# starlingonearth/MASt3R-SLAM-Quality-dualTSDF

Hardware: AMD Instinct MI355X
Metric: SLAM frames/sec (infer+match+TSDF+GN) @512x384 (higher is better)
Workload: dtype bf16

## Files before the change

mast3r-slam-quality-dualtsdf_amd/csrc/gn.hip:

```cpp
#include "common.h"
#include "sim3.h"

namespace mslam {

constexpr int kAcc = 35;
constexpr int kEdgeConst = 16;
constexpr int kPlanes = 8;
constexpr int kTile = 64;

struct GnState {
  int done;
  int iters;
  int chol_fail;
  float last_norm;
};

__device__ __forceinline__ int64_t ij_val(const int64_t* ii, const int64_t* jj, int E, int k) {
  return k < E ? ii[k] : jj[k - E];
}

__global__ __launch_bounds__(256) void gn_first_kernel(const int64_t* __restrict__ ii,
                                                       const int64_t* __restrict__ jj, int E,
                                                       int* __restrict__ first) {
  const int k = blockIdx.x * 256 + threadIdx.x;
  if (k >= 2 * E) return;
  const int64_t v = ij_val(ii, jj, E, k);
  int f = 1;
  for (int m = 0; m < k; m++)
    if (ij_val(ii, jj, E, m) == v) { f = 0; break; }
  first[k] = f;
}

__global__ __launch_bounds__(256) void gn_rank_kernel(const int64_t* __restrict__ ii,
                                                      const int64_t* __restrict__ jj, int E, int num_fix,
                                                      const int* __restrict__ first,
                                                      int* __restrict__ ii_edge, int* __restrict__ jj_edge,
                                                      int* __restrict__ ii_opt, int* __restrict__ jj_opt) {
  const int k = blockIdx.x * 256 + threadIdx.x;
  if (k >= 2 * E) return;
  const int64_t v = ij_val(ii, jj, E, k);
  int rank = 0;
  for (int m = 0; m < 2 * E; m++) rank += (first[m] && ij_val(ii, jj, E, m) < v) ? 1 : 0;
  if (k < E) { ii_edge[k] = rank; ii_opt[k] = rank - num_fix; }
  else { jj_edge[k - E] = rank; jj_opt[k - E] = rank - num_fix; }
}

__global__ void gn_edge_setup_kernel(const GnState* __restrict__ st, const float* __restrict__ Twc,
                                     const int* __restrict__ ii_edge, const int* __restrict__ jj_edge,
                                     int E, float* __restrict__ econst) {
  if (st->done) return;
  const int e = blockIdx.x * blockDim.x + threadIdx.x;
  if (e >= E) return;
  const Sim3f Ti = sim3_load(Twc + 8 * ii_edge[e]);
  const Sim3f Tj = sim3_load(Twc + 8 * jj_edge[e]);
  const Sim3f Tij = sim3_rel(Ti, Tj);
  float R[9];
  quat_to_mat(Tij.q, R);
  float* c = econst + (size_t)e * kEdgeConst;
#pragma unroll
  for (int k = 0; k < 9; k++) c[k] = Tij.s * R[k];
  c[9] = Tij.t[0]; c[10] = Tij.t[1]; c[11] = Tij.t[2];
  c[12] = c[13] = c[14] = c[15] = 0.0f;
}

__global__ __launch_bounds__(256) void gn_compact_kernel(
    const float* __restrict__ Xs, const float* __restrict__ Cs, const int* __restrict__ ii_edge,
    const int* __restrict__ jj_edge, const int64_t* __restrict__ idx_ii2jj,
    const uint8_t* __restrict__ valid_match, const float* __restrict__ Q, int num_points, int chunk_len,
    float C_thresh, float Q_thresh, float* __restrict__ stream, int* __restrict__ counts, int S, int slot_begin) {
  const int e = blockIdx.x / S, chunk = blockIdx.x - e * S;
  const int ix = ii_edge[e], jx = jj_edge[e];
  const float* __restrict__ Xi_base = Xs + (size_t)ix * num_points * 3;
  const float* __restrict__ Xj_base = Xs + (size_t)jx * num_points * 3;
  const float* __restrict__ Ci_base = Cs + (size_t)ix * num_points;
  const float* __restrict__ Cj_base = Cs + (size_t)jx * num_points;
  const int64_t* __restrict__ idx_e = idx_ii2jj + (size_t)e * num_points;
  const uint8_t* __restrict__ vm_e = valid_match + (size_t)e * num_points;
  const float* __restrict__ Q_e = Q + (size_t)e * num_points;
  float* __restrict__ slot = stream + ((size_t)(slot_begin + e) * S + chunk) * (size_t)chunk_len * kPlanes;
  __shared__ int wave_cnt[4];
  const int lane = threadIdx.x & 63, wid = threadIdx.x >> 6;
  const int k_begin = chunk * chunk_len;
  const int k_end = min(k_begin + chunk_len, num_points);
  int base = 0;
  for (int k0 = k_begin; k0 < k_end; k0 += 256) {
    const int k = k0 + (int)threadIdx.x;
    bool valid = false;
    long long ind = 0;
    float q = 0.0f;
    if (k < k_end) {
      const bool vm = vm_e[k] != 0;
      ind = vm ? idx_e[k] : 0;
      q = Q_e[k];
      const float ci = Ci_base[ind], cj = Cj_base[k];
      valid = vm & (q > Q_thresh) & (ci > C_thresh) & (cj > C_thresh);
    }
    const unsigned long long m = __ballot(valid);
    if (lane == 0) wave_cnt[wid] = __popcll(m);
    __syncthreads();
    int off = base;
    for (int w = 0; w < wid; w++) off += wave_cnt[w];
    const int total = wave_cnt[0] + wave_cnt[1] + wave_cnt[2] + wave_cnt[3];
    if (valid) {
      const int pos = off + __popcll(m & ((1ull << lane) - 1ull));
      slot[0 * (size_t)chunk_len + pos] = Xi_base[ind * 3 + 0];
      slot[1 * (size_t)chunk_len + pos] = Xi_base[ind * 3 + 1];
      slot[2 * (size_t)chunk_len + pos] = Xi_base[ind * 3 + 2];
      slot[3 * (size_t)chunk_len + pos] = Xj_base[(size_t)k * 3 + 0];
      slot[4 * (size_t)chunk_len + pos] = Xj_base[(size_t)k * 3 + 1];
      slot[5 * (size_t)chunk_len + pos] = Xj_base[(size_t)k * 3 + 2];
      slot[6 * (size_t)chunk_len + pos] = sqrtf(q);
      slot[7 * (size_t)chunk_len + pos] = __int_as_float((int)ind);
    }
    base += total;
    __syncthreads();
  }
  if (threadIdx.x == 0) counts[(slot_begin + e) * S + chunk] = base;
}

__device__ __forceinline__ float fast_rcp(float x) { return __builtin_amdgcn_rcpf(x); }
__device__ __forceinline__ float fast_rsq(float x) { return __builtin_amdgcn_rsqf(x); }

__device__ __forceinline__ float huber_w(float r) {
  return fminf(1.0f, 1.345f * fast_rcp(fabsf(r)));
}

template <unsigned NZ>
__device__ __forceinline__ void accum_row(float (&acc)[kAcc], const float (&x)[7], float w, float err) {
  const float we = w * err;
  int l = 0;
#pragma unroll
  for (int n = 0; n < 7; n++) {
    const float wx = w * x[n];
#pragma unroll
    for (int m = 0; m <= n; m++) {
      if (((NZ >> n) & 1u) && ((NZ >> m) & 1u)) acc[l] = fmaf(wx, x[m], acc[l]);
      l++;
    }
    if ((NZ >> n) & 1u) acc[28 + n] = fmaf(we, x[n], acc[28 + n]);
  }
}

struct GnParams {
  float sa_inv, sb_inv;
  float C_thresh, Q_thresh;
  int height, width;
  float border_lo, border_hi_u, border_hi_v;
  float z_eps;
  const float* K;
};

struct EdgeConst {
// ... 143 lines not shown
  }
  __syncthreads();
  if (threadIdx.x < kAcc) {
    const float s = (red[0][threadIdx.x] + red[1][threadIdx.x]) + (red[2][threadIdx.x] + red[3][threadIdx.x]);
    partial[((size_t)e * S + chunk) * kAcc + threadIdx.x] = s;
  }
}

__global__ __launch_bounds__(64) void gn_reduce_kernel(const GnState* __restrict__ st,
                                                       const float* __restrict__ partial, int S,
                                                       const float* __restrict__ Twc,
                                                       const int* __restrict__ ii_edge, int e0, int E,
                                                       float* __restrict__ Hs, float* __restrict__ gs) {
  if (st->done) return;
  const int e = blockIdx.x;
  __shared__ double B[7][7];
  __shared__ double u[7];
  __shared__ double M[7][7];
  __shared__ double MB[7][7];
  const int t = threadIdx.x;
  if (t < kAcc) {
    double s = 0.0;
    for (int c = 0; c < S; c++) s += (double)partial[((size_t)e * S + c) * kAcc + t];
    if (t < 28) {
      int n = 0, rem = t;
      while (rem > n) { rem -= n + 1; n++; }
      B[n][rem] = s;
      B[rem][n] = s;
    } else {
      u[t - 28] = s;
    }
  }
  if (t == 63) {
    const float* p = Twc + 8 * ii_edge[e];
    const double tx = p[0], ty = p[1], tz = p[2], x = p[3], y = p[4], z = p[5], w = p[6];
    const double sinv = 1.0 / (double)p[7];
    const double R[3][3] = {{1 - 2 * (y * y + z * z), 2 * (x * y - z * w), 2 * (x * z + y * w)},
                            {2 * (x * y + z * w), 1 - 2 * (x * x + z * z), 2 * (y * z - x * w)},
                            {2 * (x * z - y * w), 2 * (y * z + x * w), 1 - 2 * (x * x + y * y)}};
    for (int a = 0; a < 7; a++)
      for (int b = 0; b < 7; b++) M[a][b] = 0.0;
    for (int a = 0; a < 3; a++)
      for (int b = 0; b < 3; b++) {
        M[a][b] = sinv * R[a][b];
        M[3 + a][3 + b] = R[a][b];
      }
    for (int b = 0; b < 3; b++) {
      M[3][b] = sinv * (ty * R[2][b] - tz * R[1][b]);
      M[4][b] = sinv * (tz * R[0][b] - tx * R[2][b]);
      M[5][b] = sinv * (tx * R[1][b] - ty * R[0][b]);
      M[6][b] = sinv * (tx * R[0][b] + ty * R[1][b] + tz * R[2][b]);
    }
    M[6][6] = 1.0;
  }
  __syncthreads();
  if (t < 49) {
    const int a = t / 7, b = t % 7;
    double s = 0.0;
    for (int k = 0; k < 7; k++) s += M[a][k] * B[k][b];
    MB[a][b] = s;
  }
  __syncthreads();
  if (t < 49) {
    const int a = t / 7, b = t % 7;
    double s = 0.0;
    for (int k = 0; k < 7; k++) s += MB[a][k] * M[b][k];
    const float A = (float)s;
    const size_t o = (size_t)(e0 + e) * 49 + t;
    const size_t blk = (size_t)E * 49;
    Hs[o] = A;
    Hs[blk + o] = -A;
    Hs[2 * blk + o] = -A;
    Hs[3 * blk + o] = A;
  } else if (t < 56) {
    const int a = t - 49;
    double s = 0.0;
    for (int k = 0; k < 7; k++) s += M[a][k] * u[k];
    gs[(size_t)(e0 + e) * 7 + a] = -(float)s;
    gs[(size_t)E * 7 + (size_t)(e0 + e) * 7 + a] = (float)s;
  }
}

constexpr int kTab = 32;

__global__ __launch_bounds__(64) void gn_assemble_kernel(const GnState* __restrict__ st,
                                                         const float* __restrict__ Hs,
                                                         const float* __restrict__ gs,
                                                         const int* __restrict__ ii_opt,
                                                         const int* __restrict__ jj_opt, int E, int N,
                                                         int np, int ld, double* __restrict__ Haug,
                                                         int* __restrict__ tmin32) {
  if (st->done) return;
  const int br = blockIdx.x;
  const int lane = threadIdx.x;
  const int n = N * 7;
  if (br == N) {
    for (int r = n + lane; r < np; r += 64) {
      Haug[(size_t)r * ld + r] = 1.0;
      atomicMin(&tmin32[r >> 5], r);
    }
    if (lane == 0) tmin32[np >> 5] = 0;
    return;
  }
  int cmin = br;
  __shared__ double tab[kTab][49];
  __shared__ int tabcol[kTab];
  int ntab = 0;
  double bacc = 0.0;
  const int k7 = lane / 7, l7 = lane % 7;
  for (int blk = 0; blk < 4; blk++) {
    const int* rix = (blk < 2) ? ii_opt : jj_opt;
    const int* cix = (blk & 1) ? jj_opt : ii_opt;
    for (int e0 = 0; e0 < E; e0 += 64) {
      const int e = e0 + lane;
      const bool row_match = e < E && rix[e] == br;
      const int cj_l = row_match ? cix[e] : -1;
      unsigned long long m = __ballot(row_match);
      while (m) {
        const int b = __ffsll((long long)m) - 1;
        m &= m - 1;
        const int ee = e0 + b;
        if ((blk == 0 || blk == 2) && lane < 7)
          bacc += (double)gs[((size_t)(blk >> 1) * E + ee) * 7 + lane];
        const int cj = __shfl(cj_l, b, 64);
        if (cj < 0) continue;
        cmin = min(cmin, cj);
        const double v = lane < 49 ? (double)Hs[((size_t)blk * E + ee) * 49 + lane] : 0.0;
        const unsigned long long hit = __ballot(lane < ntab && tabcol[lane] == cj);
        int slot = hit ? __ffsll((long long)hit) - 1 : -1;
        if (slot < 0 && ntab < kTab) {
          slot = ntab++;
          if (lane == 0) tabcol[slot] = cj;
          if (lane < 49) tab[slot][lane] = 0.0;
          __builtin_amdgcn_wave_barrier();
        }
        if (lane < 49) {
          if (slot >= 0) tab[slot][lane] += v;
          else Haug[(size_t)(7 * br + k7) * ld + 7 * cj + l7] += v;
        }
      }
    }
  }
  __syncthreads();
  for (int s = 0; s < ntab; s++) {
    const int cj = tabcol[s];
    if (lane < 49) Haug[(size_t)(7 * br + k7) * ld + 7 * cj + l7] += tab[s][lane];
  }
  if (lane < 7) Haug[(size_t)np * ld + 7 * br + lane] = bacc;
  if (lane < 7) atomicMin(&tmin32[(7 * br + lane) >> 5], 7 * cmin);
}

using f64x4 = __attribute__((ext_vector_type(4))) double;

template <int NB>
__global__ __launch_bounds__(256) void chol_step_kernel(GnState* __restrict__ st, double* __restrict__ A,
                                                        double* __restrict__ Ldiag, int np, int ld, int j0,
                                                        const int* __restrict__ tmin32, int update, int clim) {
  if (st->done) return;
  constexpr int LS = NB + 2;
  constexpr int TS = kTile + 1;
  constexpr int DS = NB + 1;
  const int tj = blockIdx.x, ti = blockIdx.y;
  if (tj > ti) return;
  const int j1 = j0 + NB;
  const int r0 = j1 + ti * kTile, c0 = j1 + tj * kTile;
  if (r0 > np || c0 >= np || c0 >= clim) return;
  const bool has_update = update != 0;
  {
    const int last = np >> 5;
    const int fr = min(tmin32[min(r0 >> 5, last)], tmin32[min((r0 >> 5) + 1, last)]);
    const int fc = min(tmin32[min(c0 >> 5, last)], tmin32[min((c0 >> 5) + 1, last)]);
    if (tj != 0 && (fr >= j1 || fc >= j1)) return;
    if (tj == 0 && fr >= j1 + NB) return;
  }
  extern __shared__ double sh[];
  double* Li = sh;
  double* Lj = sh + kTile * LS;
  double* T = sh;
  double* D = sh + 2 * kTile * LS;
  double* dsave = D + NB * DS;
  double* rdiag = dsave + NB;
  __shared__ int fail;
  const int t = threadIdx.x;
  const int lane = t & 63, wid = t >> 6;
  const int wr = wid >> 1, wc = wid & 1;
  const int fcol = lane & 15, frow = lane >> 4;

  f64x4 acc[2][2];
#pragma unroll
  for (int m = 0; m < 2; m++)
#pragma unroll
    for (int n = 0; n < 2; n++)
#pragma unroll
      for (int g = 0; g < 4; g++) {
        const int r = r0 + 32 * wr + 16 * m + frow + 4 * g;
        const int c = c0 + 32 * wc + 16 * n + fcol;
        const bool in = r <= np && c < np && c <= r && c < clim;
        const double v = A[in ? (size_t)r * ld + c : (size_t)0];
        acc[m][n][g] = in ? v : 0.0;
      }
  if (has_update) {
    for (int k = t; k < kTile * NB; k += 256) {
      const int r = k / NB, q = k % NB;
      const double vi = A[(size_t)min(r0 + r, np) * ld + j0 + q];
      const double vj = A[(size_t)min(c0 + r, np) * ld + j0 + q];
      Li[r * LS + q] = (r0 + r <= np) ? vi : 0.0;
      Lj[r * LS + q] = (c0 + r < np) ? vj : 0.0;
    }
  }
  if (tj == 0) {
    for (int k = t; k < NB * NB; k += 256) {
      const int a = k / NB, b = k % NB;
      D[a * DS + b] = A[(size_t)(j1 + a) * ld + j1 + b];
    }
    if (t == 0) fail = 0;
  }
  __syncthreads();

  if (has_update) {
    if (tj == 0) {
      for (int k = t; k < NB * NB; k += 256) {
        const int a = k / NB, b = k % NB;
        if (b <= a) {
          double s = 0.0;
#pragma unroll 8
          for (int q = 0; q < NB; q++) s = fma(Lj[a * LS + q], Lj[b * LS + q], s);
          D[a * DS + b] -= s;
        }
      }
    }
    const int fi = lane & 15, fk = lane >> 4;
#pragma unroll 4
    for (int k4 = 0; k4 < NB; k4 += 4) {
      double a[2], b[2];
#pragma unroll
      for (int m = 0; m < 2; m++) {
        a[m] = -Li[(32 * wr + 16 * m + fi) * LS + k4 + fk];
        b[m] = Lj[(32 * wc + 16 * m + fi) * LS + k4 + fk];
      }
#pragma unroll
      for (int m = 0; m < 2; m++)
#pragma unroll
        for (int n = 0; n < 2; n++)
          acc[m][n] = __builtin_amdgcn_mfma_f64_16x16x4f64(a[m], b[n], acc[m][n], 0, 0, 0);
    }
  }

  if (tj != 0) {
    if (has_update) {
#pragma unroll
      for (int m = 0; m < 2; m++)
#pragma unroll
        for (int n = 0; n < 2; n++)
#pragma unroll
          for (int g = 0; g < 4; g++) {
            const int r = r0 + 32 * wr + 16 * m + frow + 4 * g;
            const int c = c0 + 32 * wc + 16 * n + fcol;
            if (r <= np && c < np && c <= r && c < clim) A[(size_t)r * ld + c] = acc[m][n][g];
          }
    }
    return;
  }

  __syncthreads();
#pragma unroll
  for (int m = 0; m < 2; m++)
#pragma unroll
    for (int n = 0; n < 2; n++)
#pragma unroll
      for (int g = 0; g < 4; g++) {
        const int rr = 32 * wr + 16 * m + frow + 4 * g;
        const int cc = 32 * wc + 16 * n + fcol;
        const int r = r0 + rr, c = c0 + cc;
        if (cc < NB) T[rr * TS + cc] = acc[m][n][g];
        else if (has_update && r <= np && c < np && c <= r && c < clim) A[(size_t)r * ld + c] = acc[m][n][g];
      }

  __syncthreads();
  for (int j = 0; j < NB; j++) {
    const double djj = D[j * DS + j];
    const bool ok = djj > 0.0;
    double d, rinv;
    if (djj > 1e-30 && djj < 1e30) {
      double r = (double)__builtin_amdgcn_rsqf((float)djj);
      const double h = 0.5 * djj;
      r = r * (1.5 - h * r * r);
      r = r * (1.5 - h * r * r);
      r = r * (1.5 - h * r * r);
      rinv = r;
      d = djj * r;
    } else {
      d = ok ? sqrt(djj) : 1.0;
      rinv = 1.0 / d;
    }
    if (t > j && t < NB) D[t * DS + j] *= rinv;
    if (t == j) {
      dsave[j] = d;
      rdiag[j] = rinv;
      if (!ok) fail = 1;
    }
    __syncthreads();
#pragma unroll
    for (int i = 0; i < NB * NB / 256; i++) {
      const int k = t + 256 * i;
      const int r = k / NB, c = k % NB;
      if (c > j && c <= r) D[r * DS + c] -= D[r * DS + j] * D[c * DS + j];
    }
    __syncthreads();
  }
  if (ti == 0) {
    if (fail && t == 0) st->chol_fail = 1;
    double* Ld = Ldiag + (size_t)(j1 / NB) * NB * NB;
    for (int k = t; k < NB * NB; k += 256) {
      const int a = k / NB, b = k % NB;
      Ld[k] = (b < a) ? D[a * DS + b] : (b == a ? dsave[a] : 0.0);
    }
  }

  if (t < kTile) {
    const int r = r0 + t;
    const bool in_diag = (ti == 0) && (t < NB);
    if (r <= np && !in_diag) {
      double x[NB];
#pragma unroll
      for (int c = 0; c < NB; c++) x[c] = T[t * TS + c];
#pragma unroll
      for (int c = 0; c < NB; c++) {
        double s = x[c];
#pragma unroll
        for (int k = 0; k < c; k++) s -= x[k] * D[c * DS + k];
        x[c] = s * rdiag[c];
      }
#pragma unroll
      for (int c = 0; c < NB; c++) T[t * TS + c] = x[c];
    }
  }
  __syncthreads();
  for (int k = t; k < kTile * NB; k += 256) {
    const int rr = k / NB, c = k % NB;
    const int r = r0 + rr;
    const bool in_diag = (ti == 0) && (rr < NB);
    if (r <= np && !in_diag) A[(size_t)r * ld + j1 + c] = T[rr * TS + c];
  }
}

__global__ __launch_bounds__(256) void chol_outer_kernel(const GnState* __restrict__ st, double* __restrict__ A, int np,
                                                         int ld, int J0, int W, const int* __restrict__ tmin32) {
  if (st->done) return;
  constexpr int KC = 32, LS = KC + 2;
  const int tj = blockIdx.x, ti = blockIdx.y;
  if (tj > ti) return;
  const int C0 = J0 + W;
  const int r0 = C0 + ti * kTile, c0 = C0 + tj * kTile;
  if (r0 > np || c0 >= np) return;
  {
    const int last = np >> 5;
    const int fr = min(tmin32[min(r0 >> 5, last)], tmin32[min((r0 >> 5) + 1, last)]);
    const int fc = min(tmin32[min(c0 >> 5, last)], tmin32[min((c0 >> 5) + 1, last)]);
    if (fr >= C0 || fc >= C0) return;
  }
  __shared__ double Li[kTile * LS], Lj[kTile * LS];
  const int t = threadIdx.x;
  const int lane = t & 63, wid = t >> 6;
  const int wr = wid >> 1, wc = wid & 1;
  const int fcol = lane & 15, frow = lane >> 4;
  f64x4 acc[2][2];
#pragma unroll
  for (int m = 0; m < 2; m++)
#pragma unroll
    for (int n = 0; n < 2; n++)
#pragma unroll
      for (int g = 0; g < 4; g++) {
        const int r = r0 + 32 * wr + 16 * m + frow + 4 * g;
        const int c = c0 + 32 * wc + 16 * n + fcol;
        const bool in = r <= np && c < np && c <= r;
        const double v = A[in ? (size_t)r * ld + c : (size_t)0];
        acc[m][n][g] = in ? v : 0.0;
      }
  const int fi = lane & 15, fk = lane >> 4;
  for (int q0 = 0; q0 < W; q0 += KC) {
    __syncthreads();
    for (int k = t; k < kTile * KC; k += 256) {
      const int r = k / KC, q = k % KC;
      const double vi = A[(size_t)min(r0 + r, np) * ld + J0 + q0 + q];
      const double vj = A[(size_t)min(c0 + r, np) * ld + J0 + q0 + q];
      Li[r * LS + q] = (r0 + r <= np) ? vi : 0.0;
      Lj[r * LS + q] = (c0 + r < np) ? vj : 0.0;
    }
    __syncthreads();
#pragma unroll 4
    for (int k4 = 0; k4 < KC; k4 += 4) {
      double a[2], b[2];
#pragma unroll
      for (int m = 0; m < 2; m++) {
        a[m] = -Li[(32 * wr + 16 * m + fi) * LS + k4 + fk];
        b[m] = Lj[(32 * wc + 16 * m + fi) * LS + k4 + fk];
      }
#pragma unroll
      for (int m = 0; m < 2; m++)
#pragma unroll
        for (int n = 0; n < 2; n++)
          acc[m][n] = __builtin_amdgcn_mfma_f64_16x16x4f64(a[m], b[n], acc[m][n], 0, 0, 0);
    }
  }
#pragma unroll
  for (int m = 0; m < 2; m++)
#pragma unroll
    for (int n = 0; n < 2; n++)
#pragma unroll
      for (int g = 0; g < 4; g++) {
        const int r = r0 + 32 * wr + 16 * m + frow + 4 * g;
        const int c = c0 + 32 * wc + 16 * n + fcol;
        if (r <= np && c < np && c <= r) A[(size_t)r * ld + c] = acc[m][n][g];
      }
}

template <int NB>
__global__ __launch_bounds__(256) void chol_back_kernel(const GnState* __restrict__ st,
                                                        double* __restrict__ A,
                                                        const double* __restrict__ Ldiag,
                                                        double* __restrict__ xs, int np, int ld, int jb) {
  if (st->done) return;
  __shared__ double Lb[NB][NB + 1];
  __shared__ double xb[NB];
  const int t = threadIdx.x;
  double* y = A + (size_t)np * ld;
  const double* Ld = Ldiag + (size_t)(jb / NB) * NB * NB;
  for (int k = t; k < NB * NB; k += 256) Lb[k / NB][k % NB] = Ld[k];
  __syncthreads();
  if (t < 64) {
    double s = t < NB ? y[jb + t] : 0.0;
    const double rd = t < NB ? 1.0 / Lb[t][t] : 0.0;
    for (int c = NB - 1; c >= 0; c--) {
      const double xc = __shfl(s * rd, c, 64);
      if (t == c) xb[c] = xc;
      if (t < c) s -= Lb[c][t] * xc;
    }
  }
  __syncthreads();
  if (blockIdx.x == 0 && t < NB) xs[jb + t] = xb[t];
  const int i = blockIdx.x * 256 + t;
  if (i < jb) {
    double s = y[i];
#pragma unroll 8
    for (int k = 0; k < NB; k++) s -= A[(size_t)(jb + k) * ld + i] * xb[k];
    y[i] = s;
  }
}

constexpr int kBackSmall = 2048;
constexpr int kOuterW = 128;
constexpr int kOuterFrom = 1536;

template <int NB>
__global__ __launch_bounds__(256) void chol_back_small_kernel(const GnState* __restrict__ st,
                                                              const double* __restrict__ A,
                                                              const double* __restrict__ Ldiag,
                                                              double* __restrict__ xs, int np, int ld) {
  if (st->done) return;
  __shared__ double ys[kBackSmall];
  __shared__ double Lb[NB][NB + 1];
  __shared__ double xb[NB];
  const int t = threadIdx.x;
  for (int i = t; i < np; i += 256) ys[i] = A[(size_t)np * ld + i];
  for (int jb = np - NB; jb >= 0; jb -= NB) {
    const double* Ld = Ldiag + (size_t)(jb / NB) * NB * NB;
    for (int k = t; k < NB * NB; k += 256) Lb[k / NB][k % NB] = Ld[k];
    __syncthreads();
    if (t < 64) {
      double s = t < NB ? ys[jb + t] : 0.0;
      const double rd = t < NB ? 1.0 / Lb[t][t] : 0.0;
      for (int c = NB - 1; c >= 0; c--) {
        const double xc = __shfl(s * rd, c, 64);
        if (t == c) xb[c] = xc;
        if (t < c) s -= Lb[c][t] * xc;
      }
    }
    __syncthreads();
    if (t < NB) xs[jb + t] = xb[t];
    for (int i = t; i < jb; i += 256) {
      double s = ys[i];
#pragma unroll 8
      for (int k = 0; k < NB; k++) s -= A[(size_t)(jb + k) * ld + i] * xb[k];
      ys[i] = s;
    }
    __syncthreads();
  }
}

__global__ __launch_bounds__(256) void gn_finish_kernel(GnState* __restrict__ st,
                                                        const double* __restrict__ xs, int N, int num_fix,
                                                        float* __restrict__ Twc, float* __restrict__ dx,
                                                        float delta_thresh) {
  if (st->done) return;
  const int t = threadIdx.x;
  const int n = N * 7;
  __shared__ float red[256];
  const bool fail = st->chol_fail != 0;
  float ss = 0.0f;
  for (int k = t; k < n; k += 256) {
    const float d = fail ? 0.0f : -(float)xs[k];
    dx[k] = d;
    ss = fmaf(d, d, ss);
  }
  red[t] = ss;
  __syncthreads();
  for (int s = 128; s > 0; s >>= 1) {
    if (t < s) red[t] += red[t + s];
    __syncthreads();
  }
  if (!fail) {
    for (int k = num_fix + t; k < N + num_fix; k += 256) {
      const Sim3f T = sim3_load(Twc + 8 * k);
      sim3_store(Twc + 8 * k, sim3_retr(dx + 7 * (k - num_fix), T));
    }
  }
  if (t == 0) {
    const float nrm = sqrtf(red[0]);
    st->last_norm = nrm;
    st->iters += 1;
    st->chol_fail = 0;
    if (nrm < delta_thresh) st->done = 1;
  }
}

__global__ void gn_state_init_kernel(GnState* st) {
  st->done = 0;
  st->iters = 0;
  st->chol_fail = 0;
  st->last_norm = 0.0f;
}

static inline size_t align_up(size_t x, size_t a) { return (x + a - 1) / a * a; }

struct GnWorkspace {
  GnState* st;
  int *ii_edge, *jj_edge, *ii_opt, *jj_opt, *first;
  float* econst;
  float* Hs;
  float* gs;
  double* Haug;
  double* Ldiag;
  double* xs;
  int* tmin32;
  int* counts;
  float* partial;
  float* stream;
  int S, chunk_len, np, ld, nb;
  size_t bytes_fixed;
  size_t bytes;
};

static GnWorkspace gn_carve(void* base, int P, int E, int HW, int local_edges) {
  GnWorkspace w;
  const int N = P > 1 ? P - 1 : 0;
  const int n = N * 7;
  w.np = (int)align_up((size_t)(n > 0 ? n : 1), kTile);
  w.ld = w.np;
  w.nb = 32;
  int S = E > 0 ? (1024 + E - 1) / E : 1;
  const int s_cap = HW / (256 * 16) > 0 ? HW / (256 * 16) : 1;
  if (S > s_cap) S = s_cap;
  if (S < 1) S = 1;
  w.S = S;
  w.chunk_len = (int)align_up((size_t)((HW + S - 1) / S), 256);
  if (w.chunk_len < 256) w.chunk_len = 256;
  size_t off = 0;
  auto take = [&](size_t bytes) { size_t o = off; off = align_up(off + bytes, 256); return (char*)base + o; };
  w.st = (GnState*)take(sizeof(GnState));
  w.ii_edge = (int*)take(sizeof(int) * (size_t)E);
  w.jj_edge = (int*)take(sizeof(int) * (size_t)E);
  w.ii_opt = (int*)take(sizeof(int) * (size_t)E);
  w.jj_opt = (int*)take(sizeof(int) * (size_t)E);
  w.first = (int*)take(sizeof(int) * 2 * (size_t)E);
  w.econst = (float*)take(sizeof(float) * (size_t)E * kEdgeConst);
  w.Hs = (float*)take(sizeof(float) * (size_t)4 * E * 49);
  w.gs = (float*)take(sizeof(float) * (size_t)2 * E * 7);
  w.Haug = (double*)take(sizeof(double) * (size_t)(w.np + 1) * w.ld);
  w.Ldiag = (double*)take(sizeof(double) * (size_t)w.np * w.nb);
  w.xs = (double*)take(sizeof(double) * (size_t)w.np);
  w.tmin32 = (int*)take(sizeof(int) * (size_t)(w.np / 32 + 2));
  w.bytes_fixed = off;
  const size_t L = local_edges > 0 ? (size_t)local_edges : 0;
  w.counts = (int*)take(sizeof(int) * L * S);
  w.partial = (float*)take(sizeof(float) * L * S * kAcc);
  w.stream = (float*)take(sizeof(float) * L * S * (size_t)w.chunk_len * kPlanes);
  w.bytes = off;
  return w;
}

static void fill_params(GnParams& P, int kind, const float* K_dev, float sigma_a, float sigma_b, int height,
                        int width, int pixel_border, float z_eps) {
  P.sa_inv = 1.0f / sigma_a;
  P.sb_inv = kind == 2 ? 0.0f : 1.0f / sigma_b;
  P.C_thresh = 0.0f;
  P.Q_thresh = 0.0f;
  P.height = height;
  P.width = width > 0 ? width : 1;
  P.border_lo = (float)pixel_border;
  P.border_hi_u = (float)(width - 1 - pixel_border);
  P.border_hi_v = (float)(height - 1 - pixel_border);
  P.z_eps = z_eps;
  P.K = K_dev;
}

static int launch_accumulate(int kind, const GnWorkspace& w, const float* Twc, int E, int e0, int cnt,
                             const GnParams& P, float* Hs, float* gs, hipStream_t s) {
  if (cnt <= 0) return MSLAM_OK;
  hipLaunchKernelGGL(gn_edge_setup_kernel, dim3((cnt + 63) / 64), dim3(64), 0, s, w.st, Twc, w.ii_edge + e0,
                     w.jj_edge + e0, cnt, w.econst);
  dim3 grid((unsigned)w.S * (unsigned)cnt);
  if (kind == 0)
    hipLaunchKernelGGL(gn_accum_kernel<0>, grid, dim3(256), 0, s, w.st, w.econst, w.stream, w.counts, w.chunk_len,
                       P, w.partial, w.S);
  else if (kind == 1)
    hipLaunchKernelGGL(gn_accum_kernel<1>, grid, dim3(256), 0, s, w.st, w.econst, w.stream, w.counts, w.chunk_len,
                       P, w.partial, w.S);
  else
    hipLaunchKernelGGL(gn_accum_kernel<2>, grid, dim3(256), 0, s, w.st, w.econst, w.stream, w.counts, w.chunk_len,
                       P, w.partial, w.S);
  hipLaunchKernelGGL(gn_reduce_kernel, dim3(cnt), dim3(64), 0, s, w.st, w.partial, w.S, Twc, w.ii_edge + e0, e0, E,
                     Hs, gs);
  return check_hip(hipGetLastError(), "gn accumulate launch");
}

template <int NB>
static int launch_cholesky(const GnWorkspace& w, hipStream_t s) {
  constexpr size_t shmem = sizeof(double) * (2 * kTile * (NB + 2) + NB * (NB + 1) + 2 * NB);
  static bool attr_set = false;
  if (shmem > 48 * 1024 && !attr_set) {
    int rc = check_hip(hipFuncSetAttribute((const void*)chol_step_kernel<NB>,
                                           hipFuncAttributeMaxDynamicSharedMemorySize, (int)shmem),
                       "hipFuncSetAttribute(chol_step)");
    if (rc) return rc;
    attr_set = true;
  }
  auto step = [&](int j0, int update, int clim) {
    const int j1 = j0 + NB;
    const int tiles_r = (w.np - j1 + 1 + kTile - 1) / kTile;
    const int cend = clim < w.np ? clim : w.np;
    const int tiles_c = update ? (cend - j1 + kTile - 1) / kTile : 1;
    hipLaunchKernelGGL(chol_step_kernel<NB>, dim3(tiles_c > 0 ? tiles_c : 1, tiles_r), dim3(256), shmem, s, w.st, w.Haug,
                       w.Ldiag, w.np, w.ld, j0, w.tmin32, update, clim);
  };
  const int W = w.np > kOuterFrom ? kOuterW : w.np;
  step(-NB, 0, w.np);
  for (int J0 = 0; J0 < w.np; J0 += W) {
    const int jend = J0 + W < w.np ? J0 + W : w.np;
    for (int j0 = J0; j0 + NB < jend; j0 += NB) step(j0, 1, jend);
    if (jend < w.np) {
      const int tiles = (w.np - jend + 1 + kTile - 1) / kTile;
      hipLaunchKernelGGL(chol_outer_kernel, dim3((w.np - jend + kTile - 1) / kTile, tiles), dim3(256), 0, s, w.st, w.Haug,
                         w.np, w.ld, J0, jend - J0, w.tmin32);
      step(jend - NB, 0, w.np);
    }
  }
  if (w.np <= kBackSmall) {
    hipLaunchKernelGGL(chol_back_small_kernel<NB>, dim3(1), dim3(256), 0, s, w.st, w.Haug, w.Ldiag, w.xs, w.np, w.ld);
  } else {
    for (int jb = w.np - NB; jb >= 0; jb -= NB) {
      const int blocks = jb > 0 ? (jb + 255) / 256 : 1;
      hipLaunchKernelGGL(chol_back_kernel<NB>, dim3(blocks), dim3(256), 0, s, w.st, w.Haug, w.Ldiag, w.xs, w.np,
                         w.ld, jb);
    }
  }
  return MSLAM_OK;
}

static int launch_solve(const GnWorkspace& w, const float* Hs, const float* gs, int E, int P, float* Twc,
                        float* dx, float delta_thresh, hipStream_t s) {
  const int N = P - 1;
  int rc = check_hip(hipMemsetAsync(w.Haug, 0, sizeof(double) * (size_t)(w.np + 1) * w.ld, s), "Haug memset");
  if (rc) return rc;
  rc = check_hip(hipMemsetAsync(w.tmin32, 0x7f, sizeof(int) * (size_t)(w.np / 32 + 2), s), "tmin32 memset");
  if (rc) return rc;
  hipLaunchKernelGGL(gn_assemble_kernel, dim3(N + 1), dim3(64), 0, s, w.st, Hs, gs, w.ii_opt, w.jj_opt, E, N, w.np,
                     w.ld, w.Haug, w.tmin32);
  rc = launch_cholesky<32>(w, s);
  if (rc) return rc;
  hipLaunchKernelGGL(gn_finish_kernel, dim3(1), dim3(256), 0, s, w.st, w.xs, N, 1, Twc, dx, delta_thresh);
  return check_hip(hipGetLastError(), "gn solve launch");
}

static int gn_check_ws(size_t need, void* workspace, size_t workspace_bytes, const char* who) {
  if (!workspace || need > workspace_bytes) {
    set_error("%s: workspace too small (%zu < %zu)", who, workspace ? workspace_bytes : (size_t)0, need);
    return MSLAM_ENOMEM;
  }
  return MSLAM_OK;
}

}

using namespace mslam;

extern "C" size_t mslam_gn_workspace_bytes(int num_poses, int num_edges, int num_points, int local_edges) {
  if (num_poses < 0 || num_edges < 0 || num_points < 0 || local_edges < 0) return 0;
  return gn_carve(nullptr, num_poses, num_edges, num_points, local_edges).bytes;
}

extern "C" int mslam_gn_begin(const int64_t* ii, const int64_t* jj, int num_poses, int num_edges,
                              int num_points, void* workspace, size_t workspace_bytes, void* stream) {
  MSLAM_REQUIRE(num_poses >= 2 && num_edges >= 1, "gn_begin: need >= 2 poses and >= 1 edge");
  MSLAM_REQUIRE(ii && jj, "gn_begin: null pointer");
  MSLAM_REQUIRE(num_edges <= (1 << 22), "gn_begin: %d edges (the index preparation is quadratic in the edge count)", num_edges);
  GnWorkspace w = gn_carve(workspace, num_poses, num_edges, num_points, 0);
  int rc = gn_check_ws(w.bytes_fixed, workspace, workspace_bytes, "gn_begin");
  if (rc) return rc;
  hipStream_t s = (hipStream_t)stream;
  const int blocks = (2 * num_edges + 255) / 256;
  hipLaunchKernelGGL(gn_state_init_kernel, dim3(1), dim3(1), 0, s, w.st);
  hipLaunchKernelGGL(gn_first_kernel, dim3(blocks), dim3(256), 0, s, ii, jj, num_edges, w.first);
  hipLaunchKernelGGL(gn_rank_kernel, dim3(blocks), dim3(256), 0, s, ii, jj, num_edges, 1, w.first, w.ii_edge,
                     w.jj_edge, w.ii_opt, w.jj_opt);
  return check_hip(hipGetLastError(), "gn_begin launch");
}

extern "C" int mslam_gn_compact_at(const float* Xs, const float* Cs, const int64_t* idx_ii2jj,
                                   const uint8_t* valid_match, const float* Q, int num_poses, int num_points,
                                   int num_edges, int edge_begin, int edge_count, int slot_begin, int range_count,
                                   float C_thresh, float Q_thresh, void* workspace, size_t workspace_bytes,
                                   void* stream) {
  MSLAM_REQUIRE(num_poses >= 2 && num_points >= 1 && num_edges >= 1, "gn_compact: bad sizes");
  MSLAM_REQUIRE(edge_begin >= 0 && edge_count >= 0 && edge_begin + edge_count <= num_edges,
                "gn_compact: edge range [%d,%d) outside [0,%d)", edge_begin, edge_begin + edge_count, num_edges);
  MSLAM_REQUIRE(slot_begin >= 0 && slot_begin + edge_count <= range_count,
                "gn_compact: slots [%d,%d) outside the accumulate range of %d edges", slot_begin,
                slot_begin + edge_count, range_count);
  if (edge_count == 0) return MSLAM_OK;
  MSLAM_REQUIRE(Xs && Cs && idx_ii2jj && valid_match && Q, "gn_compact: null pointer");
  GnWorkspace w = gn_carve(workspace, num_poses, num_edges, num_points, range_count);
  int rc = gn_check_ws(w.bytes, workspace, workspace_bytes, "gn_compact");
  if (rc) return rc;
  hipLaunchKernelGGL(gn_compact_kernel, dim3((unsigned)w.S * (unsigned)edge_count), dim3(256), 0, (hipStream_t)stream, Xs,
                     Cs, w.ii_edge + edge_begin, w.jj_edge + edge_begin, idx_ii2jj, valid_match, Q, num_points,
                     w.chunk_len, C_thresh, Q_thresh, w.stream, w.counts, w.S, slot_begin);
  return check_hip(hipGetLastError(), "gn_compact launch");
}

extern "C" int mslam_gn_compact(const float* Xs, const float* Cs, const int64_t* idx_ii2jj,
                                const uint8_t* valid_match, const float* Q, int num_poses, int num_points,
                                int num_edges, int edge_begin, int edge_count, float C_thresh, float Q_thresh,
                                void* workspace, size_t workspace_bytes, void* stream) {
  return mslam_gn_compact_at(Xs, Cs, idx_ii2jj, valid_match, Q, num_poses, num_points, num_edges, edge_begin,
                             edge_count, 0, edge_count, C_thresh, Q_thresh, workspace, workspace_bytes, stream);
}

extern "C" int mslam_gn_accumulate(int kind, const float* Twc, const float* K, int num_poses, int num_points,
                                   int num_edges, int edge_begin, int edge_count, float sigma_a, float sigma_b,
                                   int height, int width, int pixel_border, float z_eps, float* Hs, float* gs,
                                   void* workspace, size_t workspace_bytes, void* stream) {
  MSLAM_REQUIRE(kind >= 0 && kind <= 2, "gn_accumulate: kind must be 0 (rays), 1 (calib) or 2 (points)");
  MSLAM_REQUIRE(num_poses >= 2 && num_points >= 1 && num_edges >= 1, "gn_accumulate: bad sizes");
  MSLAM_REQUIRE(edge_begin >= 0 && edge_count >= 0 && edge_begin + edge_count <= num_edges,
                "gn_accumulate: edge range [%d,%d) outside [0,%d)", edge_begin, edge_begin + edge_count, num_edges);
  if (edge_count == 0) return MSLAM_OK;
  MSLAM_REQUIRE(Twc && Hs && gs, "gn_accumulate: null pointer");
  MSLAM_REQUIRE(kind != 1 || (K && width > 0 && height > 0), "gn_accumulate: calib needs K, height, width");
  GnWorkspace w = gn_carve(workspace, num_poses, num_edges, num_points, edge_count);
  int rc = gn_check_ws(w.bytes, workspace, workspace_bytes, "gn_accumulate");
  if (rc) return rc;
  GnParams P;
  fill_params(P, kind, K, sigma_a, sigma_b, height, width, pixel_border, z_eps);
  return launch_accumulate(kind, w, Twc, num_edges, edge_begin, edge_count, P, Hs, gs, (hipStream_t)stream);
}

extern "C" int mslam_gn_solve_retract(const float* Hs, const float* gs, int num_poses, int num_edges,
                                      int num_points, float* Twc, float* dx, float delta_thresh,
                                      void* workspace, size_t workspace_bytes, void* stream) {
  MSLAM_REQUIRE(num_poses >= 2 && num_edges >= 1, "gn_solve_retract: need >= 2 poses and >= 1 edge");
  MSLAM_REQUIRE(Hs && gs && Twc && dx, "gn_solve_retract: null pointer");
  GnWorkspace w = gn_carve(workspace, num_poses, num_edges, num_points, 0);
  int rc = gn_check_ws(w.bytes_fixed, workspace, workspace_bytes, "gn_solve_retract");
  if (rc) return rc;
  return launch_solve(w, Hs, gs, num_edges, num_poses, Twc, dx, delta_thresh, (hipStream_t)stream);
}

extern "C" int mslam_gn_status(int* status4, int num_poses, int num_edges, int num_points, void* workspace,
                               size_t workspace_bytes, void* stream) {
  MSLAM_REQUIRE(status4, "gn_status: null pointer");
  GnWorkspace w = gn_carve(workspace, num_poses, num_edges, num_points, 0);
  int rc = gn_check_ws(w.bytes_fixed, workspace, workspace_bytes, "gn_status");
  if (rc) return rc;
  return check_hip(hipMemcpyAsync(status4, w.st, sizeof(GnState), hipMemcpyDeviceToDevice, (hipStream_t)stream),
                   "gn_status copy");
}

static int gauss_newton_impl(int kind, float* Twc, const float* Xs, const float* Cs, const float* K,
                             const int64_t* ii, const int64_t* jj, const int64_t* idx_ii2jj,
                             const uint8_t* valid_match, const float* Q, int num_poses, int num_points,
                             int num_edges, float sigma_a, float sigma_b, float C_thresh, float Q_thresh,
                             int height, int width, int pixel_border, float z_eps, int max_iter,
                             float delta_thresh, float* dx, void* workspace, size_t workspace_bytes,
                             void* stream) {
  MSLAM_REQUIRE(num_poses >= 2, "gauss_newton: need at least 2 poses (got %d)", num_poses);
  MSLAM_REQUIRE(num_edges >= 1 && num_points >= 1, "gauss_newton: need at least one edge and one point");
  MSLAM_REQUIRE(Twc && Xs && Cs && ii && jj && idx_ii2jj && valid_match && Q && dx, "gauss_newton: null pointer");
  MSLAM_REQUIRE(kind != 1 || (K && width > 0 && height > 0), "gauss_newton_calib needs K, height, width");
  int rc = mslam_gn_begin(ii, jj, num_poses, num_edges, num_points, workspace, workspace_bytes, stream);
  if (rc) return rc;
  rc = mslam_gn_compact(Xs, Cs, idx_ii2jj, valid_match, Q, num_poses, num_points, num_edges, 0, num_edges, C_thresh,
                        Q_thresh, workspace, workspace_bytes, stream);
  if (rc) return rc;
  GnWorkspace w = gn_carve(workspace, num_poses, num_edges, num_points, num_edges);
  hipStream_t s = (hipStream_t)stream;
  GnParams P;
  fill_params(P, kind, K, sigma_a, sigma_b, height, width, pixel_border, z_eps);
  rc = check_hip(hipMemsetAsync(dx, 0, sizeof(float) * 7 * (size_t)(num_poses - 1), s), "dx memset");
  if (rc) return rc;
  for (int it = 0; it < max_iter; it++) {
    rc = launch_accumulate(kind, w, Twc, num_edges, 0, num_edges, P, w.Hs, w.gs, s);
    if (rc) return rc;
    rc = launch_solve(w, w.Hs, w.gs, num_edges, num_poses, Twc, dx, delta_thresh, s);
    if (rc) return rc;
  }
  return MSLAM_OK;
}

extern "C" int mslam_gauss_newton_rays(float* Twc, const float* Xs, const float* Cs, const int64_t* ii,
                                       const int64_t* jj, const int64_t* idx_ii2jj, const uint8_t* valid_match,
                                       const float* Q, int num_poses, int num_points, int num_edges,
                                       float sigma_ray, float sigma_dist, float C_thresh, float Q_thresh,
                                       int max_iter, float delta_thresh, float* dx, void* workspace,
                                       size_t workspace_bytes, void* stream) {
  return gauss_newton_impl(0, Twc, Xs, Cs, nullptr, ii, jj, idx_ii2jj, valid_match, Q, num_poses, num_points,
                           num_edges, sigma_ray, sigma_dist, C_thresh, Q_thresh, 0, 0, 0, 0.0f, max_iter,
                           delta_thresh, dx, workspace, workspace_bytes, stream);
}

extern "C" int mslam_gauss_newton_calib(float* Twc, const float* Xs, const float* Cs, const float* K,
// ... 75 lines not shown
```

Baseline: 161.6.

## Fuse blocked Cholesky, back-substitution and update into one single-block kernel

For systems with up to 1024 unknowns, the multi-launch blocked Cholesky, triangular solve and finish kernels are replaced by one 512-thread single-workgroup kernel. It factors the diagonal block in one wave, does the panel solve per row, and applies the trailing update with f64 MFMA tiles while skipping structurally empty tiles. Back-substitution and the pose update run inside the same kernel, and an environment variable restores the old panel path. The aim is to remove many small kernel launches and their gaps, at the cost of running the factorization on a single compute unit.

```diff
diff --git a/mast3r-slam-quality-dualtsdf_amd/csrc/gn.hip b/mast3r-slam-quality-dualtsdf_amd/csrc/gn.hip
--- a/mast3r-slam-quality-dualtsdf_amd/csrc/gn.hip
+++ b/mast3r-slam-quality-dualtsdf_amd/csrc/gn.hip
@@ -1,3 +1,6 @@
+#include <stdlib.h>
+#include <string.h>
+
 #include "common.h"
 #include "sim3.h"
 
@@ -447,6 +450,23 @@
 
 using f64x4 = __attribute__((ext_vector_type(4))) double;
 
+__device__ __forceinline__ bool chol_pivot(double djj, double& d, double& rinv) {
+  const bool ok = djj > 0.0;
+  if (djj > 1e-30 && djj < 1e30) {
+    double r = (double)__builtin_amdgcn_rsqf((float)djj);
+    const double h = 0.5 * djj;
+    r = r * (1.5 - h * r * r);
+    r = r * (1.5 - h * r * r);
+    r = r * (1.5 - h * r * r);
+    rinv = r;
+    d = djj * r;
+  } else {
+    d = ok ? sqrt(djj) : 1.0;
+    rinv = 1.0 / d;
+  }
+  return ok;
+}
+
 template <int NB>
 __global__ __launch_bounds__(256) void chol_step_kernel(GnState* __restrict__ st, double* __restrict__ A,
                                                         double* __restrict__ Ldiag, int np, int ld, int j0,
@@ -573,21 +593,8 @@
 
   __syncthreads();
   for (int j = 0; j < NB; j++) {
-    const double djj = D[j * DS + j];
-    const bool ok = djj > 0.0;
     double d, rinv;
-    if (djj > 1e-30 && djj < 1e30) {
-      double r = (double)__builtin_amdgcn_rsqf((float)djj);
-      const double h = 0.5 * djj;
-      r = r * (1.5 - h * r * r);
-      r = r * (1.5 - h * r * r);
-      r = r * (1.5 - h * r * r);
-      rinv = r;
-      d = djj * r;
-    } else {
-      d = ok ? sqrt(djj) : 1.0;
-      rinv = 1.0 / d;
-    }
+    const bool ok = chol_pivot(D[j * DS + j], d, rinv);
     if (t > j && t < NB) D[t * DS + j] *= rinv;
     if (t == j) {
       dsave[j] = d;
@@ -783,28 +790,26 @@
   }
 }
 
-__global__ __launch_bounds__(256) void gn_finish_kernel(GnState* __restrict__ st,
-                                                        const double* __restrict__ xs, int N, int num_fix,
-                                                        float* __restrict__ Twc, float* __restrict__ dx,
-                                                        float delta_thresh) {
-  if (st->done) return;
+__device__ __forceinline__ void gn_finish_block(GnState* __restrict__ st, const double* xs, bool fail, int N,
+                                                int num_fix, float* __restrict__ Twc, float* __restrict__ dx,
+                                                float delta_thresh, float* red) {
   const int t = threadIdx.x;
   const int n = N * 7;
-  __shared__ float red[256];
-  const bool fail = st->chol_fail != 0;
   float ss = 0.0f;
-  for (int k = t; k < n; k += 256) {
-    const float d = fail ? 0.0f : -(float)xs[k];
-    dx[k] = d;
-    ss = fmaf(d, d, ss);
-  }
-  red[t] = ss;
+  if (t < 256) {
+    for (int k = t; k < n; k += 256) {
+      const float d = fail ? 0.0f : -(float)xs[k];
+      dx[k] = d;
+      ss = fmaf(d, d, ss);
+    }
+    red[t] = ss;
+  }
   __syncthreads();
   for (int s = 128; s > 0; s >>= 1) {
     if (t < s) red[t] += red[t + s];
     __syncthreads();
   }
-  if (!fail) {
+  if (!fail && t < 256) {
     for (int k = num_fix + t; k < N + num_fix; k += 256) {
       const Sim3f T = sim3_load(Twc + 8 * k);
       sim3_store(Twc + 8 * k, sim3_retr(dx + 7 * (k - num_fix), T));
@@ -817,6 +822,190 @@
     st->chol_fail = 0;
     if (nrm < delta_thresh) st->done = 1;
   }
+}
+
+__global__ __launch_bounds__(256) void gn_finish_kernel(GnState* __restrict__ st,
+                                                        const double* __restrict__ xs, int N, int num_fix,
+                                                        float* __restrict__ Twc, float* __restrict__ dx,
+                                                        float delta_thresh) {
+  if (st->done) return;
+  __shared__ float red[256];
+  gn_finish_block(st, xs, st->chol_fail != 0, N, num_fix, Twc, dx, delta_thresh, red);
+}
+
+constexpr int kFusedMax = 1024;
+constexpr int kFusedThreads = 512;
+
+__device__ __forceinline__ double readlane_f64(double v, int l) {
+  const unsigned long long b = (unsigned long long)__double_as_longlong(v);
+  const unsigned lo = (unsigned)__builtin_amdgcn_readlane((int)(unsigned)b, l);
+  const unsigned hi = (unsigned)__builtin_amdgcn_readlane((int)(unsigned)(b >> 32), l);
+  return __longlong_as_double((long long)(((unsigned long long)hi << 32) | lo));
+}
+
+__device__ __forceinline__ void wave_lds_sync() {
+  __builtin_amdgcn_fence(__ATOMIC_SEQ_CST, "wavefront");
+  __builtin_amdgcn_wave_barrier();
+}
+
+__global__ __launch_bounds__(kFusedThreads) void gn_solve_fused_kernel(GnState* __restrict__ st,
+                                                                       double* __restrict__ A,
+                                                                       double* __restrict__ xs, int np, int ld,
+                                                                       const int* __restrict__ tmin32, int N,
+                                                                       float* __restrict__ Twc,
+                                                                       float* __restrict__ dx, float delta_thresh) {
+  if (st->done) return;
+  constexpr int NB = 32, DS = NB + 1, NW = kFusedThreads / 64;
+  __shared__ double L11[NB * DS];
+  __shared__ double rdiag[NB];
+  __shared__ double ys[kFusedMax];
+  __shared__ double xb[NB];
+  __shared__ float red[256];
+  __shared__ int fail;
+  const int t = threadIdx.x;
+  const int lane = t & 63, wid = t >> 6;
+  const int last = np >> 5;
+  if (t == 0) fail = 0;
+
+  for (int j0 = 0; j0 < np; j0 += NB) {
+    const int j1 = j0 + NB;
+    if (wid == 0) {
+      for (int k = lane; k < NB * NB; k += 64) {
+        const int r = k >> 5, c = k & 31;
+        L11[r * DS + c] = c <= r ? A[(size_t)(j0 + r) * ld + j0 + c] : 0.0;
+      }
+      wave_lds_sync();
+      bool bad = false;
+      for (int j = 0; j < NB; j++) {
+        double d, rinv;
+        bad |= !chol_pivot(L11[j * DS + j], d, rinv);
+        if (lane > j && lane < NB) L11[lane * DS + j] *= rinv;
+        if (lane == j) { L11[j * DS + j] = d; rdiag[j] = rinv; }
+        wave_lds_sync();
+#pragma unroll
+        for (int i = 0; i < NB * NB / 64; i++) {
+          const int k = lane + 64 * i;
+          const int r = k >> 5, c = k & 31;
+          if (c > j && c <= r) L11[r * DS + c] -= L11[r * DS + j] * L11[c * DS + j];
+        }
+        wave_lds_sync();
+      }
+      for (int k = lane; k < NB * NB; k += 64) {
+        const int r = k >> 5, c = k & 31;
+        if (c <= r) A[(size_t)(j0 + r) * ld + j0 + c] = L11[r * DS + c];
+      }
+      if (bad && lane == 0) fail = 1;
+    }
+    __syncthreads();
+    for (int r = j1 + t; r <= np; r += kFusedThreads) {
+      if (tmin32[r >> 5] >= j1) continue;
+      double* row = A + (size_t)r * ld + j0;
+      double x[NB];
+#pragma unroll
+      for (int c = 0; c < NB; c++) x[c] = row[c];
+#pragma unroll
+      for (int c = 0; c < NB; c++) {
+        double s = x[c];
+#pragma unroll
+        for (int k = 0; k < c; k++) s -= x[k] * L11[c * DS + k];
+        x[c] = s * rdiag[c];
+        __builtin_amdgcn_sched_barrier(0);
+      }
+#pragma unroll
+      for (int c = 0; c < NB; c++) row[c] = x[c];
+    }
+    __syncthreads();
+    const int b1 = j1 >> 5;
+    const int nrb = last - b1 + 1;
+    const int ntiles = nrb * (nrb + 1) / 2;
+    const int fi = lane & 15, fk = lane >> 4;
+    const int fcol = lane & 15, frow = lane >> 4;
+    for (int q = wid; q < ntiles; q += NW) {
+      int a = (int)((sqrtf(8.0f * (float)q + 1.0f) - 1.0f) * 0.5f);
+      while (a * (a + 1) / 2 > q) a--;
+      while ((a + 1) * (a + 2) / 2 <= q) a++;
+      const int rb = b1 + a, cb = b1 + (q - a * (a + 1) / 2);
+      if (cb >= last) continue;
+      if (tmin32[rb] >= j1 || tmin32[cb] >= j1) continue;
+      const int r0 = rb * 32, c0 = cb * 32;
+      f64x4 acc[2][2];
+#pragma unroll
+      for (int m = 0; m < 2; m++)
+#pragma unroll
+        for (int n = 0; n < 2; n++)
+#pragma unroll
+          for (int g = 0; g < 4; g++) {
+            const int r = r0 + 16 * m + frow + 4 * g, c = c0 + 16 * n + fcol;
+            const bool in = r <= np && c <= r;
+            const double v = A[in ? (size_t)r * ld + c : (size_t)0];
+            acc[m][n][g] = in ? v : 0.0;
+          }
+      const double* Li[2];
+      const double* Lj[2];
+      bool li_in[2];
+#pragma unroll
+      for (int m = 0; m < 2; m++) {
+        const int ri = r0 + 16 * m + fi;
+        li_in[m] = ri <= np;
+        Li[m] = A + (size_t)(li_in[m] ? ri : np) * ld + j0 + fk;
+        Lj[m] = A + (size_t)(c0 + 16 * m + fi) * ld + j0 + fk;
+      }
+#pragma unroll
+      for (int k4 = 0; k4 < NB; k4 += 4) {
+        double av[2], bv[2];
+#pragma unroll
+        for (int m = 0; m < 2; m++) {
+          av[m] = li_in[m] ? -Li[m][k4] : 0.0;
+          bv[m] = Lj[m][k4];
+        }
+#pragma unroll
+        for (int m = 0; m < 2; m++)
+#pragma unroll
+          for (int n = 0; n < 2; n++)
+            acc[m][n] = __builtin_amdgcn_mfma_f64_16x16x4f64(av[m], bv[n], acc[m][n], 0, 0, 0);
+      }
+#pragma unroll
+      for (int m = 0; m < 2; m++)
+#pragma unroll
+        for (int n = 0; n < 2; n++)
+#pragma unroll
+          for (int g = 0; g < 4; g++) {
+            const int r = r0 + 16 * m + frow + 4 * g, c = c0 + 16 * n + fcol;
+            if (r <= np && c <= r) A[(size_t)r * ld + c] = acc[m][n][g];
+          }
+    }
+    __syncthreads();
+  }
+
+  for (int i = t; i < np; i += kFusedThreads) ys[i] = A[(size_t)np * ld + i];
+  for (int jb = np - NB; jb >= 0; jb -= NB) {
+    __syncthreads();
+    if (wid == 0) {
+      const int l = lane & 31;
+      double lc[NB];
+#pragma unroll
+      for (int c = 0; c < NB; c++) lc[c] = A[(size_t)(jb + c) * ld + jb + l];
+      double s = lane < NB ? ys[jb + lane] : 0.0;
+      const double rd = 1.0 / A[(size_t)(jb + l) * ld + jb + l];
+#pragma unroll
+      for (int c = NB - 1; c >= 0; c--) {
+        const double xc = readlane_f64(s * rd, c);
+        if (lane == c) xb[c] = xc;
+        if (lane < c) s -= lc[c] * xc;
+      }
+    }
+    __syncthreads();
+    if (t < NB) { xs[jb + t] = xb[t]; ys[jb + t] = xb[t]; }
+    const int lo = min(tmin32[jb >> 5], jb) & ~31;
+    for (int i = lo + t; i < jb; i += kFusedThreads) {
+      double s = ys[i];
+#pragma unroll 8
+      for (int k = 0; k < NB; k++) s -= A[(size_t)(jb + k) * ld + i] * xb[k];
+      ys[i] = s;
+    }
+  }
+  __syncthreads();
+  gn_finish_block(st, ys, fail != 0, N, 1, Twc, dx, delta_thresh, red);
 }
 
 __global__ void gn_state_init_kernel(GnState* st) {
@@ -962,6 +1151,11 @@
   return MSLAM_OK;
 }
 
+static bool gn_force_panel() {
+  const char* e = getenv("MSLAM_GN_SOLVE");
+  return e && strcmp(e, "panel") == 0;
+}
+
 static int launch_solve(const GnWorkspace& w, const float* Hs, const float* gs, int E, int P, float* Twc,
                         float* dx, float delta_thresh, hipStream_t s) {
   const int N = P - 1;
@@ -971,6 +1165,11 @@
   if (rc) return rc;
   hipLaunchKernelGGL(gn_assemble_kernel, dim3(N + 1), dim3(64), 0, s, w.st, Hs, gs, w.ii_opt, w.jj_opt, E, N, w.np,
                      w.ld, w.Haug, w.tmin32);
+  if (w.np <= kFusedMax && !gn_force_panel()) {
+    hipLaunchKernelGGL(gn_solve_fused_kernel, dim3(1), dim3(kFusedThreads), 0, s, w.st, w.Haug, w.xs, w.np, w.ld,
+                       w.tmin32, N, Twc, dx, delta_thresh);
+    return check_hip(hipGetLastError(), "gn solve launch");
+  }
   rc = launch_cholesky<32>(w, s);
   if (rc) return rc;
   hipLaunchKernelGGL(gn_finish_kernel, dim3(1), dim3(256), 0, s, w.st, w.xs, N, 1, Twc, dx, delta_thresh);
```

New measurement: 145.7, median of 2. 0.901x the previous value.
